# unsynchronized/gr-amps

Hardware: AMD Instinct MI355X
Metric: AMPS RECC Manchester symbols demodulated+decoded per second (real-time channels = value/0.02); achieved HBM GB/s vs peak (higher is better)
Workload: dtype f32

## Files before the change

gr_amps_amd/csrc/recc_decode.hip.h:

```cpp
#pragma once
#include <hip/hip_runtime.h>
#include <stdint.h>
#include "amps_recc.h"
#include "amps_recc_numerics.h"
#include "recc_devmem.hip.h"
#include "recc_record_host.h"

namespace amps {

struct Gf64Tables {
    uint8_t exp[128];
    uint8_t log[64];
};
constexpr Gf64Tables make_gf64()
{
    Gf64Tables t{};
    unsigned v = 1;
    for (int i = 0; i < 63; i++) {
        t.exp[i] = (uint8_t)v;
        t.exp[i + 63] = (uint8_t)v;
        t.log[v] = (uint8_t)i;
        v <<= 1;
        if (v & 0x40) v ^= 0x43;
    }
    t.exp[126] = t.exp[0];
    t.exp[127] = t.exp[1];
    t.log[0] = 0;
    return t;
}
struct SynMasks { uint64_t m1[6], m3[6]; };
constexpr SynMasks make_syn_masks()
{
    SynMasks s{};
    const Gf64Tables t = make_gf64();
    for (int e = 0; e < 63; e++)
        for (int k = 0; k < 6; k++) {
            if ((t.exp[e] >> k) & 1) s.m1[k] |= 1ull << e;
            if ((t.exp[(3 * e) % 63] >> k) & 1) s.m3[k] |= 1ull << e;
        }
    return s;
}
static constexpr SynMasks k_syn = make_syn_masks();

__device__ __forceinline__ unsigned gf_xtime(unsigned a)
{
    a <<= 1;
    return a ^ ((a & 0x40u) ? 0x43u : 0u);
}
__device__ __forceinline__ unsigned gf_mul(unsigned a, unsigned b)
{
    unsigned r = 0;
#pragma unroll
    for (int i = 0; i < 6; i++) { r ^= ((b >> i) & 1u) ? a : 0u; a = gf_xtime(a); }
    return r;
}
__device__ __forceinline__ unsigned gf_inv(unsigned a)
{
    const unsigned a2 = gf_mul(a, a), a4 = gf_mul(a2, a2), a8 = gf_mul(a4, a4), a16 = gf_mul(a8, a8), a32 = gf_mul(a16, a16);
    return gf_mul(gf_mul(gf_mul(a2, a4), gf_mul(a8, a16)), a32);
}
__device__ __forceinline__ unsigned gf_div(unsigned a, unsigned b) { return gf_mul(a, gf_inv(b)); }

struct BchResult {
    int ok;
    int nflip;
    int e[3];
};

__device__ __forceinline__ BchResult bch63_decode_packed(uint64_t w)
{
    BchResult r;
    r.ok = 0; r.nflip = 0; r.e[0] = r.e[1] = r.e[2] = -1;
    unsigned S1 = 0, S3 = 0;
#pragma unroll
    for (int k = 0; k < 6; k++) {
        S1 |= (unsigned)(__popcll(w & k_syn.m1[k]) & 1) << k;
        S3 |= (unsigned)(__popcll(w & k_syn.m3[k]) & 1) << k;
    }
    if ((S1 | S3) == 0) { r.ok = 1; return r; }
    int found = 0, e0 = -1, e1 = -1, e2 = -1;
    auto take = [&](bool root, int j) {
        const int pos = (63 - j) % 63;
        e0 = (root && found == 0) ? pos : e0;
        e1 = (root && found == 1) ? pos : e1;
        e2 = (root && found == 2) ? pos : e2;
        found += (root && found < 3) ? 1 : 0;
    };
    if (S1 != 0) {
        const unsigned S1cube = gf_mul(gf_mul(S1, S1), S1);
        const unsigned delta = S3 ^ S1cube;
        if (delta == 0) {
            unsigned p = 1;
            int lg = 0;
#pragma unroll 1
            for (int j = 0; j < 63; j++) { if (p == S1) lg = j; p = gf_xtime(p); }
            r.ok = 1; r.nflip = 1; r.e[0] = lg;
            return r;
        }
        const unsigned c2 = gf_div(delta, S1);
        unsigned a = S1, b = c2;
#pragma unroll 1
        for (int j = 0; j < 63; j++) {
            take((1u ^ a ^ b) == 0, j);
            a = gf_xtime(a);
            b = gf_xtime(gf_xtime(b));
        }
        r.e[0] = e0; r.e[1] = e1; r.e[2] = e2;
        if (found == 2) { r.ok = 1; r.nflip = 2; }
        return r;
    }
    {
        unsigned c = S3;
#pragma unroll 1
        for (int j = 0; j < 63; j++) {
            take((1u ^ c) == 0, j);
            c = gf_xtime(gf_xtime(gf_xtime(c)));
        }
        r.e[0] = e0; r.e[1] = e1; r.e[2] = e2;
        if (found == 3) { r.ok = 1; r.nflip = 3; }
    }
    return r;
}

__device__ __forceinline__ BchResult bch_short_decode(const uint8_t *bits, int nbits)
{
    uint64_t w = 0;
    for (int i = 0; i < nbits; i++) w |= (uint64_t)(bits[i] & 1u) << (nbits - 1 - i);
    return bch63_decode_packed(w);
}

__device__ __forceinline__ BchResult bch4836_decode(const uint8_t *bits) { return bch_short_decode(bits, 48); }

__device__ __forceinline__ BchResult bch4836_decode_aligned(const uint8_t *bits)
{
    const uint64_t *p = (const uint64_t *)bits;
    uint64_t w = 0;
#pragma unroll
    for (int c = 0; c < 6; c++) w |= ((p[c] * 0x8040201008040201ull) >> 56) << (40 - 8 * c);
    return bch63_decode_packed(w);
}

__device__ __forceinline__ void bch_short_encode(const uint8_t *msg, int k, uint8_t *cw)
{
    unsigned rem = 0;
    for (int j = 0; j < k; j++) {
        unsigned fb = ((rem >> 11) & 1u) ^ (msg[j] & 1u);
        rem = (rem << 1) & 0xfffu;
        if (fb) rem ^= 0x539u;
        cw[j] = msg[j] & 1u;
    }
    for (int j = 0; j < 12; j++) cw[k + j] = (uint8_t)((rem >> (11 - j)) & 1u);
}

__device__ __forceinline__ unsigned getbits(const uint8_t *b, int n)
{
    unsigned v = 0;
    for (int i = 0; i < n; i++) v = (v << 1) | (b[i] & 1u);
    return v;
}

__device__ __forceinline__ void extract_min_3(unsigned val, char *out)
{
    unsigned m2 = val + 111;
    unsigned dig = m2 % 10;
    out[2] = (char)('0' + dig);
    if (dig == 0) m2 -= 10; else m2 -= dig;
    dig = (m2 % 100) / 10;
    out[1] = (char)('0' + dig);
    if (dig == 0) m2 -= 100; else m2 -= (m2 % 100);
    dig = m2 / 100;
    if (dig > 9) dig = 0;
    out[0] = (char)('0' + dig);
}

constexpr int BOFF = 1;
struct DecodeCore {
    alignas(8) uint8_t bits[1696];
    uint64_t packed[7];
    uint32_t bad[8];
    uint32_t nonbin;
    int8_t   ok[35];
    int8_t   flip[35][3];
    int8_t   rr[8];
    int8_t   dly[AMPS_TRACK_BLOCKS];
    amps_recc_burst_t rec;
};
struct DecodeScratch {
    DecodeCore k;
    uint8_t sym[AMPS_RECC_CAPTURE_SYMS + 2];
};

struct BlockSync { static __device__ __forceinline__ void sync() { __syncthreads(); } };
struct WaveSync {
    static __device__ __forceinline__ void sync()
    {
        __builtin_amdgcn_fence(__ATOMIC_RELEASE, "wavefront");
        __builtin_amdgcn_wave_barrier();
        __builtin_amdgcn_fence(__ATOMIC_ACQUIRE, "wavefront");
    }
};

__device__ __forceinline__ void decode_core_begin(DecodeCore &s, int lane)
{
    if (lane < 8) s.bad[lane] = 0;
    if (lane == 8) s.nonbin = 0;
    for (int i = lane; i < (int)(sizeof(amps_recc_burst_t) / 4); i += 64) ((uint32_t *)&s.rec)[i] = 0;
}

template <class Sync>
__device__ __forceinline__ void manchester_from_sym(DecodeCore &s, const uint8_t *sym, int lane)
{
    decode_core_begin(s, lane);
    Sync::sync();
    const uint16_t *s16 = (const uint16_t *)sym;
#pragma unroll 9
    for (int it = 0; it < 27; it++) {
        const int k = lane + 64 * it;
        if (k < 1687) {
            const unsigned pr = s16[k];
            const unsigned sa = pr & 0xffu, sb = pr >> 8;
            const bool nonbin = (sa | sb) > 1u;
            const bool same = sa == sb;
            const unsigned bit = nonbin ? 0u : (same ? (sa ^ 1u) : sb);
            s.bits[BOFF + k] = (uint8_t)bit;
            if (nonbin) atomicOr(&s.nonbin, 1u);
            if (nonbin || same) atomicAdd(&s.bad[k < 7 ? 0 : 1 + (k - 7) / 240], 1u);
        }
    }
    Sync::sync();
}

constexpr int TRACK_PRE_BITS = AMPS_RECC_TRIGGER_SYMS / 2;
__host__ __device__ constexpr uint32_t capture_lead(uint32_t sps) { return sps * (AMPS_RECC_TRIGGER_SYMS - 1) + AMPS_TRACK_BLOCKS; }
__device__ __forceinline__ uint64_t capture_first_word(uint64_t nc, uint32_t sps)
{
    const uint64_t lead = capture_lead(sps);
    return (nc > lead ? nc - lead : 0ull) >> 6;
}
__device__ __forceinline__ uint32_t wave_sum_u32(uint32_t v)
{
    v += (uint32_t)__builtin_amdgcn_update_dpp(0, (int)v, 0xB1, 0xf, 0xf, true);
    v += (uint32_t)__builtin_amdgcn_update_dpp(0, (int)v, 0x4E, 0xf, 0xf, true);
    v += (uint32_t)__builtin_amdgcn_update_dpp(0, (int)v, 0x124, 0xf, 0xf, true);
    v += (uint32_t)__builtin_amdgcn_update_dpp(0, (int)v, 0x128, 0xf, 0xf, true);
    v += (uint32_t)__builtin_amdgcn_update_dpp(0, (int)v, 0x142, 0xa, 0xf, false);
    v += (uint32_t)__builtin_amdgcn_update_dpp(0, (int)v, 0x143, 0xc, 0xf, false);
    return (uint32_t)__builtin_amdgcn_readlane((int)v, 63);
}
template <class Sync, bool TWO = false>
__device__ __forceinline__ void manchester_from_ring(DecodeCore &s, const uint64_t *ring, uint64_t nc, uint64_t w0, uint32_t sps, int lane, bool track,
                                                     bool keep_delays = true)
{
    constexpr int EARLY = TWO ? 2 : 1;
    decode_core_begin(s, lane);
    Sync::sync();
    const uint32_t *r32 = (const uint32_t *)ring;
    const int32_t base = (int32_t)(nc - (w0 << 6));
    const uint32_t midmask = (1u << (sps - 1)) - 1u;
    uint32_t f_lo = 0u, f_hi = 0u, f_sh = 0u;
    int dly = 0, dly_fetched = 0;
    uint32_t badacc = 0u;
    auto fetch = [&](int k, int d, bool on) {
        const uint32_t na = (uint32_t)(base + (int32_t)sps * (2 * k + 1) + d - EARLY);
        const uint32_t q = on ? na >> 5 : 0u;
        f_lo = r32[q]; f_hi = r32[q + 1]; f_sh = na & 31u;
    };
    auto measure = [&](uint32_t w, bool on) {
        const uint32_t sa = w & 1u, sb = (w >> sps) & 1u;
        const uint32_t mid = (w >> 1) & midmask;
        const uint32_t cnt = (uint32_t)__popc(sa ? mid : (~mid & midmask));
        const uint32_t contrib = (on && sa != sb) ? ((cnt | (1u << 10)) << (sa ? 0 : 16)) : 0u;
        const uint32_t tot = wave_sum_u32(contrib);
        const int sum1 = (int)(tot & 0x3ffu), n1 = (int)((tot >> 10) & 0x3fu), sum0 = (int)((tot >> 16) & 0x3ffu), n0 = (int)(tot >> 26);
        const int E1 = 2 * sum1 - (int)(sps - 1) * n1, E0 = 2 * sum0 - (int)(sps - 1) * n0;
        const int lhs = E1 * n0 + E0 * n1, rhs = 2 * n0 * n1;
        if (rhs > 0) dly += lhs > rhs ? 1 : lhs < -rhs ? -1 : 0;
    };
    auto choose2 = [&](uint32_t w, bool on) -> int {
        const uint32_t e = w ^ (w >> 2);
        const uint32_t contrib = on ? ((~e & 1u) | ((~e & 2u) << 7) | ((~e & 4u) << 14)) : 0u;
        const uint32_t tot = wave_sum_u32(contrib);
        const uint32_t vm = tot & 0xffu, v0 = (tot >> 8) & 0xffu, vp = tot >> 16;
        int mv = 0;
        uint32_t best = v0;
        if (vm < v0) { mv = -1; best = vm; }
        if (vp < v0 && vp < best) mv = 1;
        return mv;
    };
    {
        const int k = -TRACK_PRE_BITS + lane;
        const bool on = lane < TRACK_PRE_BITS;
        const int32_t nas = base + (int32_t)sps * (2 * k + 1) - 1;
        const uint32_t na = nas < 0 ? 0u : (uint32_t)nas, q = on ? na >> 5 : 0u;
        const int32_t sh = -nas - 1;
        const uint32_t w = nas >= 0 ? __builtin_amdgcn_alignbit(r32[q + 1], r32[q], na & 31u) >> 1
                                    : sh >= 32 ? ~0u : ((r32[0] << (uint32_t)sh) | ((1u << (uint32_t)sh) - 1u));
        fetch(lane, 0, lane < 7 + AMPS_RECC_WORD_BITS);
        if constexpr (TWO) {
            const uint32_t w2 = nas >= 0 ? __builtin_amdgcn_alignbit(r32[q + 1], r32[q], na & 31u)
                                         : sh + 1 >= 32 ? ~0u : ((r32[0] << (uint32_t)(sh + 1)) | ((1u << (uint32_t)(sh + 1)) - 1u));
            if (track) dly += choose2(w2, on);
            if (lane == 0 && keep_delays) s.dly[0] = (int8_t)dly;
        } else {
        if (lane == 0 && keep_delays) s.dly[0] = 0;
        if (track) measure(w, on);
        }
    }
    {
        const int k = lane;
        const bool on = lane < 7 + AMPS_RECC_WORD_BITS;
        uint32_t w = __builtin_amdgcn_alignbit(f_hi, f_lo, f_sh) >> (uint32_t)(dly + 1);
        const int d1 = dly;
        fetch(7 + AMPS_RECC_WORD_BITS + lane, d1, lane < AMPS_RECC_WORD_BITS);
        if constexpr (TWO) {
            const int mv = track ? choose2(w, on) : 0;
            dly += mv;
            w >>= (uint32_t)(mv + 1);
        }
        if (lane == 0 && keep_delays) s.dly[1] = (int8_t)dly;
        const uint32_t sa = w & 1u, sb = (w >> sps) & 1u;
        if (on) s.bits[BOFF + k] = (uint8_t)(sa == sb ? (sa ^ 1u) : sb);
        const uint64_t bad = __ballot(on && sa == sb);
        if (lane == 0) s.bad[0] = (uint32_t)__popcll(bad & 0x7full);
        badacc = (uint32_t)__popcll(bad >> 7);
        if constexpr (!TWO) { if (track) measure(w, on); }
        dly_fetched = d1;
    }
    const bool on48 = lane < AMPS_RECC_WORD_BITS;
    uint8_t *bitp = &s.bits[BOFF + 7 + AMPS_RECC_WORD_BITS + lane];
    int kn = 7 + 2 * AMPS_RECC_WORD_BITS + lane;
    int rep = 1, word = 0;
#pragma unroll 1
    for (int b = 2; b < AMPS_TRACK_BLOCKS; b++) {
        uint32_t w = __builtin_amdgcn_alignbit(f_hi, f_lo, f_sh) >> (uint32_t)(dly - dly_fetched + 1);
        dly_fetched = dly;
        fetch(kn, dly, on48 && b + 1 < AMPS_TRACK_BLOCKS);
        kn += AMPS_RECC_WORD_BITS;
        if constexpr (TWO) {
            const int mv = track ? choose2(w, on48) : 0;
            dly += mv;
            w >>= (uint32_t)(mv + 1);
        }
        if (lane == 0 && keep_delays) s.dly[b] = (int8_t)dly;
        const uint32_t sa = w & 1u, sb = (w >> sps) & 1u;
        if (on48) *bitp = (uint8_t)(sa == sb ? (sa ^ 1u) : sb);
        bitp += AMPS_RECC_WORD_BITS;
        badacc += (uint32_t)__popcll(__ballot(on48 && sa == sb));
        if (++rep == AMPS_RECC_REPEATS) {
            if (lane == 0) s.bad[1 + word] = badacc;
            badacc = 0u; rep = 0; word++;
        }
        if constexpr (!TWO) { if (track) measure(w, on48); }
    }
    Sync::sync();
}

__device__ __forceinline__ void decode_core_store(const DecodeCore &s, amps_recc_burst_t *__restrict__ out, int lane)
{
    for (int i = lane; i < (int)(sizeof(amps_recc_burst_t) / 4); i += 64) ((uint32_t *)out)[i] = ((const uint32_t *)&s.rec)[i];
}

__device__ __forceinline__ void decode_core_store_packed(const DecodeCore &s, uint32_t *__restrict__ out, int lane)
{
    const uint32_t *rec = (const uint32_t *)&s.rec;
    if (lane < PACKED_RECORD_BYTES / 4) {
        uint32_t v;
        if (lane < 13) v = rec[lane];
        else if (lane >= 32) v = rec[REC_TAIL_OFF / 4 + (lane - 32)];
        else {
            const uint32_t *src = rec + (lane < 24 ? REC_RAW_OFF / 4 + 8 * (lane - 13) : REC_DEC_OFF / 4 + 8 * (lane - 24));
            v = 0u;
#pragma unroll
            for (int j = 0; j < 8; j++) {
                v |= ((((src[j] & 0x01010101u) * 0x01020408u) >> 24) & 0xfu) << (4 * j);
            }
        }
        out[lane] = v;
    }
}

struct NoTl { __device__ __forceinline__ void mark(int) {} };
template <class Sync, class Tl = NoTl>
__device__ __forceinline__ void decode_core_wave(DecodeCore &s, uint32_t channel, uint64_t position,
                                                 amps_recc_burst_t *__restrict__ out, bool majority, int lane, Tl tl = Tl())
{
    amps_recc_burst_t &o = s.rec;
    if (!majority) {
        if (lane < 35) {
            const int w = lane / 5, r = lane % 5;
            BchResult br = bch4836_decode_aligned(&s.bits[BOFF + 7 + 240 * w + 48 * r]);
            s.ok[lane] = (int8_t)br.ok;
            s.flip[lane][0] = (int8_t)br.e[0];
            s.flip[lane][1] = (int8_t)br.e[1];
            s.flip[lane][2] = (int8_t)br.e[2];
        }
        Sync::sync();
        tl.mark(1);
        if (lane < 7) {
            const int w = lane;
            int r = 0, ok = 0;
            for (; r < 5; r++) if (s.ok[w * 5 + r]) { ok = 1; break; }
            o.valid[w] = (uint8_t)ok;
            o.first_valid_rep[w] = (uint8_t)r;
            o.manch_bad[w] = (uint16_t)s.bad[1 + w];
            s.rr[w] = (int8_t)(ok ? r : 4);
        }
        for (int i = lane; i < 7 * 48; i += 64) o.word_raw[i / 48][i % 48] = s.bits[BOFF + 7 + 240 * (i / 48) + (i % 48)];
        Sync::sync();
        tl.mark(2);
        for (int i = lane; i < 7 * 36; i += 64) {
            const int w = i / 36, b = i % 36;
            o.word_dec[w][b] = s.bits[BOFF + 7 + 240 * w + 48 * s.rr[w] + b];
        }
        Sync::sync();
        tl.mark(3);
        if (lane < 7 && o.valid[lane]) {
            const int w = lane;
            for (int f = 0; f < 3; f++) {
                int e = s.flip[w * 5 + s.rr[w]][f];
                if (e >= 12 && e <= 47) o.word_dec[w][47 - e] ^= 1u;
            }
        }
    } else {
        for (int i = lane; i < 7 * 48; i += 64) {
            const int w = i / 48, b = i % 48;
            int cnt = 0;
            for (int r = 0; r < 5; r++) cnt += s.bits[BOFF + 7 + 240 * w + 48 * r + b];
            o.word_raw[w][b] = (uint8_t)(cnt >= 3);
        }
        Sync::sync();
        if (lane < 7) {
            const int w = lane;
            BchResult br = bch4836_decode(o.word_raw[w]);
            int ok = br.ok;
            for (int f = 0; f < 3; f++) if (br.e[f] >= 48) ok = 0;
            o.valid[w] = (uint8_t)ok;
            int agree = 0;
            for (int r = 0; r < 5; r++) {
                unsigned diff = 0;
#pragma unroll 8
                for (int b = 0; b < 48; b++) diff |= (unsigned)(s.bits[BOFF + 7 + 240 * w + 48 * r + b] ^ o.word_raw[w][b]);
                agree += diff == 0;
            }
            o.first_valid_rep[w] = (uint8_t)agree;
            o.manch_bad[w] = (uint16_t)s.bad[1 + w];
            for (int i = 0; i < 36; i++) o.word_dec[w][i] = o.word_raw[w][i];
            if (ok) for (int f = 0; f < 3; f++) { int e = br.e[f]; if (e >= 12 && e <= 47) o.word_dec[w][47 - e] ^= 1u; }
        }
    }
    if (lane < 7) o.dcc[lane] = s.bits[BOFF + lane];
    Sync::sync();
    tl.mark(4);
    for (int w = 0; w < 7; w++) {
        const uint8_t *src = majority ? o.word_dec[w] : o.word_raw[w];
        const unsigned bit = lane < 36 ? (src[lane] & 1u) : 0u;
        const uint64_t m = __ballot(bit != 0);
        if (lane == 0) s.packed[w] = __brevll(m);
    }
    Sync::sync();
    tl.mark(5);

    if (lane == 0) {
        o.channel = channel;
        o.position = position;
        o.flags = s.nonbin ? AMPS_BURST_FLAG_NONBINARY : 0u;
        o.dcc_bad = (uint8_t)s.bad[0];
        bool used_ok = true;
        auto W = [&](int w) -> uint64_t { used_ok = used_ok && o.valid[w]; return s.packed[w]; };
        auto fld = [](uint64_t wp, int off, int n) -> unsigned { return (unsigned)((wp >> (64 - off - n)) & ((1ull << n) - 1ull)); };
        const uint64_t A = W(0), B = W(1);
        if (majority) {
            const unsigned d = getbits(o.dcc, 7);
            const bool good = __popc(d ^ 0x00u) <= 1 || __popc(d ^ 0x1fu) <= 1 || __popc(d ^ 0x63u) <= 1 || __popc(d ^ 0x7cu) <= 1;
            if (!good) o.flags |= AMPS_BURST_FLAG_DCC_INVALID;
        }
        o.a_F = (uint8_t)fld(A, 0, 1); o.a_NAWC = (uint8_t)fld(A, 1, 3);
        o.a_T = (uint8_t)fld(A, 4, 1); o.a_S = (uint8_t)fld(A, 5, 1); o.a_E = (uint8_t)fld(A, 6, 1); o.a_ER = (uint8_t)fld(A, 7, 1);
        o.a_SCM = (uint8_t)fld(A, 8, 4); o.a_MIN1 = fld(A, 12, 24);
        o.b_F = (uint8_t)fld(B, 0, 1); o.b_NAWC = (uint8_t)fld(B, 1, 3);
        o.b_MSG_TYPE = (uint8_t)fld(B, 4, 5); o.b_ORDQ = (uint8_t)fld(B, 9, 3);
        o.b_ORDER = (uint8_t)fld(B, 12, 5); o.b_LT = (uint8_t)fld(B, 17, 1); o.b_EP = (uint8_t)fld(B, 18, 1);
        o.b_SCM4 = (uint8_t)fld(B, 19, 1); o.b_MPCI = (uint8_t)fld(B, 20, 2); o.b_SDCC1 = (uint8_t)fld(B, 22, 2);
        o.b_SDCC2 = (uint8_t)fld(B, 24, 2); o.b_MIN2 = (uint16_t)fld(B, 26, 10);
        extract_min_3(o.b_MIN2, o.min);
        extract_min_3((o.a_MIN1 >> 14) & 0x3ff, o.min + 3);
        unsigned thous = (o.a_MIN1 >> 10) & 0xf;
        if (thous > 9) thous = 0;
        o.min[6] = (char)('0' + thous);
        extract_min_3(o.a_MIN1 & 0x3ff, o.min + 7);

        const bool zero_order = (o.b_ORDER == 0 && o.b_ORDQ == 0 && o.b_MSG_TYPE == 0);
        if (!o.valid[0]) o.msg_class = AMPS_MSG_INVALID_WORD_A;
        else if (!o.a_E) o.msg_class = AMPS_MSG_E_ZERO;
        else if (o.a_T == 0 && zero_order) o.msg_class = AMPS_MSG_PAGE_RESPONSE;
        else if (o.a_T == 1 && o.b_ORDER == 0xd) {
            o.msg_class = AMPS_MSG_REGISTRATION;
            o.has_esn = o.a_S;
            if (o.a_S && o.a_NAWC > 1) {
                const uint64_t Cw = W(2);
                o.esn = fld(Cw, 4, 32);
                uint8_t nawc = (uint8_t)(o.a_NAWC - 2);
                if ((uint8_t)fld(Cw, 1, 3) != nawc) o.flags |= AMPS_BURST_FLAG_WORDC_NAWC_MISMATCH;
            }
        } else if (o.a_T == 1 && (o.a_NAWC > 2 || zero_order)) {
            uint8_t nawc = o.a_NAWC;
            unsigned next = 2;
            o.has_esn = o.a_S;
            if (o.a_S) {
                const uint64_t Cw = W(next++);
                o.esn = fld(Cw, 4, 32);
                nawc = (uint8_t)(o.a_NAWC - 2);
                if ((uint8_t)fld(Cw, 1, 3) != nawc) o.flags |= AMPS_BURST_FLAG_WORDC_NAWC_MISMATCH;
            }
            if (nawc < 1 || nawc > 4) o.msg_class = AMPS_MSG_BAD_NAWC;
            else {
                o.msg_class = AMPS_MSG_ORIGINATION;
                int dl = 0;
                for (; nawc > 0; nawc--) {
                    unsigned digs = fld(W(next++), 4, 32);
                    for (int i = 0; i < 8; i++) {
                        unsigned v = (digs >> 28) & 0xf;
                        if (v == 0) break;
                        if (v >= 13) { o.flags |= AMPS_BURST_FLAG_BAD_DIGIT; break; }
                        o.dialed[dl++] = v <= 9 ? (char)('0' + v) : v == 10 ? '0' : v == 11 ? '*' : '#';
                        digs <<= 4;
                    }
                    o.n_called_words++;
                }
            }
        } else o.msg_class = AMPS_MSG_UNKNOWN;
        if (majority && !used_ok && o.msg_class >= AMPS_MSG_PAGE_RESPONSE) o.msg_class = AMPS_MSG_INVALID_WORD_A;
    }
    Sync::sync();
    tl.mark(6);
    if (out) decode_core_store(s, out, lane);
    tl.mark(7);
}

__device__ __forceinline__ void decode_burst_wave(DecodeScratch &s, uint32_t channel, uint64_t position,
                                                  amps_recc_burst_t *__restrict__ out, bool majority = false)
{
    const int lane = threadIdx.x & 63;
    manchester_from_sym<BlockSync>(s.k, s.sym, lane);
    decode_core_wave<BlockSync>(s.k, channel, position, out, majority, lane);
}

__global__ __launch_bounds__(256) void bch_encode_words_kernel(const uint8_t *msg, uint32_t n, int k, uint8_t *cw)
{
    for (uint32_t i = blockIdx.x * 256 + threadIdx.x; i < n; i += gridDim.x * 256) {
        unsigned rem = 0;
        for (int j = 0; j < k; j++) {
            const unsigned bit = msg[(uint64_t)i * k + j] & 1u;
            const unsigned fb = ((rem >> 11) & 1u) ^ bit;
            rem = (rem << 1) & 0xfffu;
            if (fb) rem ^= 0x539u;
            cw[(uint64_t)i * (k + 12) + j] = (uint8_t)bit;
        }
        for (int j = 0; j < 12; j++) cw[(uint64_t)i * (k + 12) + k + j] = (uint8_t)((rem >> (11 - j)) & 1u);
    }
}
__global__ __launch_bounds__(256) void bch_decode_words_kernel(const uint8_t *cw, uint32_t n, int k, uint8_t *msg, uint8_t *valid,
                                                               uint8_t *nerr)
{
    const int nb = k + 12;
    for (uint32_t i = blockIdx.x * 256 + threadIdx.x; i < n; i += gridDim.x * 256) {
        uint64_t w = 0;
        for (int j = 0; j < nb; j++) w |= (uint64_t)(cw[(uint64_t)i * nb + j] & 1u) << (nb - 1 - j);
        const uint64_t raw = w;
        BchResult r = bch63_decode_packed(w);
        int ok = r.ok;
#pragma unroll
        for (int f = 0; f < 3; f++) {
            const int e = r.e[f];
            if (e >= nb) ok = 0;
            else if (r.ok && e >= 0) w ^= 1ull << e;
        }
        const uint64_t out = ok ? w : raw;
        for (int j = 0; j < k; j++) msg[(uint64_t)i * k + j] = (uint8_t)((out >> (nb - 1 - j)) & 1ull);
        valid[i] = (uint8_t)ok;
        nerr[i] = (uint8_t)(ok ? r.nflip : 0xff);
    }
}

struct BchScratch { DevBuf<uint8_t> in, out, val, err; };
inline int bch_grow(DevBuf<uint8_t> &b, size_t need)
{
    if (need <= b.capacity()) return 0;
    return b.reserve(need < 4096 ? 4096 : need + need / 2);
}
inline int bch_stage_in(BchScratch &b, hipStream_t s, const uint8_t *in, size_t nin, int mem, const uint8_t **din)
{
    if (mem == AMPS_MEM_DEVICE) { *din = in; return 0; }
    if (int rc = bch_grow(b.in, nin)) return rc;
    if (hipMemcpyAsync(b.in.get(), in, nin, hipMemcpyHostToDevice, s) != hipSuccess) return -EIO;
    *din = b.in.get();
    return 0;
}

}
```

gr_amps_amd/csrc/recc_resolve.hip.h:

```cpp
#pragma once
#include "recc_decode.hip.h"
#include "recc_bits.hip.h"

namespace amps {

struct ResolveArgs {
    const uint64_t *det;
    const uint32_t *detcount;
    uint32_t max_chunks, det_cap;
    uint32_t tiles_per_channel, span;
    uint32_t sps;
    uint64_t n_proc;
    uint64_t *next_allowed;
    uint64_t *pending;
    uint32_t *status;
    const uint64_t *gring;
    uint32_t ring_mask, ring_words;
    uint32_t cap_words;
    amps_recc_burst_t *records;
    uint32_t *nrecords;
    uint32_t rec_cap;
    uint32_t majority;
    uint32_t track;
    uint8_t *burst_syms;
    unsigned long long *done_blocks;
    uint32_t *hdr_host;
    uint64_t *capq;
    uint32_t *capq_count;
    uint32_t capq_cap;
    uint32_t search_P;
    uint32_t search_tol;
    uint32_t *zero1, *zero2;
    unsigned long long *tl;
};
#ifdef RESOLVE_TIMELINE
#define RTL(k) do { if (a.tl && tid == 0) a.tl[(size_t)blockIdx.x * 24 + (k)] = __builtin_amdgcn_s_memtime(); } while (0)
#else
#define RTL(k) do { } while (0)
#endif

constexpr int CAP_WAVES = 4;
__host__ __device__ constexpr uint32_t resolve_cap_stride(uint32_t cap_words) { return (uint32_t)((sizeof(DecodeCore) + 7) / 8) + cap_words; }
inline uint32_t resolve_cap_words(uint32_t sps) { return (AMPS_RECC_CAPTURE_SYMS * sps + sps + capture_lead(sps) + AMPS_TRACK_BLOCKS) / 64 + 4; }
inline size_t resolve_dyn_lds(uint32_t sps) { return (size_t)CAP_WAVES * resolve_cap_stride(resolve_cap_words(sps)) * 8; }

#ifdef RESOLVE_TIMELINE
struct RtlStamps {
    unsigned long long *dst;
    __device__ __forceinline__ void mark(int k) { if (dst) dst[k] = __builtin_amdgcn_s_memtime(); }
};
#else
typedef NoTl RtlStamps;
#endif
__device__ __forceinline__ void capture_gather_wave(const ResolveArgs &a, uint32_t c, uint64_t nc, uint64_t *scratch, int lane, RtlStamps tl = RtlStamps())
{
    uint64_t *s_ring = scratch + (sizeof(DecodeCore) + 7) / 8;
    const uint64_t *ring = a.gring + (uint64_t)c * a.ring_words;
    const uint64_t w0 = capture_first_word(nc, a.sps);
    const int nw = (int)(((nc + (uint64_t)a.sps * (AMPS_RECC_CAPTURE_SYMS + 1) + AMPS_TRACK_BLOCKS + 32) >> 6) - w0) + 1;
    for (int i0 = 0; i0 < nw; i0 += 512) {
        uint64_t v[8];
#pragma unroll
        for (int u = 0; u < 8; u++) {
            const int i = i0 + 64 * u + lane;
            v[u] = i < nw ? ring[(w0 + (uint64_t)i) & a.ring_mask] : 0ull;
        }
#pragma unroll
        for (int u = 0; u < 8; u++) {
            const int i = i0 + 64 * u + lane;
            if (i < nw) s_ring[i] = v[u];
        }
    }
    WaveSync::sync();
    tl.mark(8);
}
template <bool TWO>
__device__ __forceinline__ void capture_decode_wave(const ResolveArgs &a, uint32_t c, uint64_t nc, uint64_t *scratch, int lane, RtlStamps tl = RtlStamps())
{
    DecodeCore &k = *(DecodeCore *)scratch;
    const uint64_t *s_ring = scratch + (sizeof(DecodeCore) + 7) / 8;
    const uint64_t w0 = capture_first_word(nc, a.sps);
    manchester_from_ring<WaveSync, TWO>(k, s_ring, nc, w0, a.sps, lane, a.track != 0, a.burst_syms != nullptr);
    tl.mark(0);
    decode_core_wave<WaveSync>(k, c, nc, nullptr, a.majority != 0, lane, tl);
}
__device__ __forceinline__ void capture_store_wave(const ResolveArgs &a, uint64_t nc, uint32_t slot, const uint64_t *scratch, int lane)
{
    const DecodeCore &k = *(const DecodeCore *)scratch;
    decode_core_store_packed(k, (uint32_t *)((uint8_t *)a.records + (size_t)slot * PACKED_RECORD_BYTES), lane);
    if (a.burst_syms) {
        const uint64_t *s_ring = scratch + (sizeof(DecodeCore) + 7) / 8;
        const uint64_t w0 = capture_first_word(nc, a.sps);
        uint32_t *dst = (uint32_t *)(a.burst_syms + (uint64_t)slot * PACKED_BURST_BYTES);
        for (int dw = lane; dw < PACKED_BURST_BYTES / 4; dw += 64) {
            uint32_t word = 0u;
            for (int j = 0; j < 32; j++) {
                const int i = 32 * dw + j;
                if (i < AMPS_RECC_CAPTURE_SYMS) {
                    const int kb = i >> 1, blk = kb < 7 + AMPS_RECC_WORD_BITS ? 1 : 2 + (kb - 7 - AMPS_RECC_WORD_BITS) / AMPS_RECC_WORD_BITS;
                    const uint64_t n = (uint64_t)((int64_t)nc + (int64_t)a.sps * (i + 1) + k.dly[blk]);
                    word |= (uint32_t)((s_ring[(n >> 6) - w0] >> (n & 63)) & 1ull) << j;
                }
            }
            dst[dw] = word;
        }
    }
}

constexpr uint32_t DONE_GROUPS = 32;
__device__ __forceinline__ unsigned long long count_done(unsigned long long *p, uint32_t done, unsigned long long reserved)
{
    return __hip_atomic_fetch_add(p, (reserved << 32) | done, __ATOMIC_RELAXED, __HIP_MEMORY_SCOPE_AGENT);
}
__device__ __forceinline__ void publish_header(uint32_t *nrecords , uint32_t *status,
                                               volatile uint32_t *hdr_host, unsigned long long launch_total)
{
    const uint32_t total = nrecords[2] + (uint32_t)launch_total;
    nrecords[2] = total;
    hdr_host[0] = total;
    hdr_host[1] = __hip_atomic_load(status, __ATOMIC_RELAXED, __HIP_MEMORY_SCOPE_AGENT);
}

constexpr int RESOLVE_THREADS = 256;
constexpr int RESOLVE_THREADS_WIDE = 1024;
constexpr int RESOLVE_LDS_HITS = 512;
constexpr int RESOLVE_LDS_HITS_WIDE = 2048;

constexpr int RESOLVE_SEARCH_CAP = 320;
template <int THREADS, int HITS, bool TWO = false, int SEARCH = 0, bool STOL = false>
__global__ __launch_bounds__(THREADS, 4) void recc_resolve_kernel(ResolveArgs a)
{
    static_assert(SEARCH == 0 || (THREADS == 256 && (SEARCH == 2 || SEARCH == 3)), "the search stage runs in the narrow kernel, at the wideband seam's rates");
    __shared__ __attribute__((aligned(16))) uint32_t s_sw[SEARCH ? 4 : 1][SEARCH ? 8 + 64 * 4 : 1];
    __shared__ uint64_t s_sdet[SEARCH ? 4 : 1][SEARCH ? RESOLVE_SEARCH_CAP : 1];
    __shared__ uint32_t s_scnt[4];
    __shared__ uint64_t s_hits[HITS];
    __shared__ uint32_t s_scan[THREADS / 64];
    __shared__ uint64_t s_acc[HITS + 1];
    __shared__ uint8_t  s_head[HITS], s_accf[HITS];
    __shared__ uint64_t s_na_out, s_pend;
    __shared__ uint32_t s_total, s_nacc, s_base;
    extern __shared__ uint64_t s_cap[];
    const int c = blockIdx.x, tid = threadIdx.x;
    const int wv = __builtin_amdgcn_readfirstlane(tid >> 6), lane = tid & 63;
    RTL(0);
    const uint64_t span_hold = (uint64_t)a.sps * (AMPS_RECC_CAPTURE_SYMS + AMPS_RECC_TRIGGER_SYMS);
    const uint64_t span_done = (uint64_t)a.sps * (AMPS_RECC_CAPTURE_SYMS + 1) + (a.track ? AMPS_TRACK_BLOCKS : 0);
    uint64_t next_allowed = a.next_allowed[c];
    uint64_t pend = a.pending[c];
    if constexpr (SEARCH != 0) {
        if (blockIdx.x == 0 && tid == 0) {
            if (a.zero1) *a.zero1 = 0u;
            if (a.zero2) { a.zero2[0] = 0u; a.zero2[1] = 0u; a.zero2[2] = 0u; }
        }
        const uint32_t Tc = (a.search_P + TILE - 1) / TILE;
        const uint32_t t_lo = (uint32_t)((uint64_t)Tc * (uint32_t)wv / 4u), t_hi = (uint32_t)((uint64_t)Tc * ((uint32_t)wv + 1u) / 4u);
        uint32_t nd = 0;
        if (t_hi > t_lo)
            nd = bits_search_segment<SEARCH, STOL>(a.gring + (uint64_t)c * a.ring_words, a.ring_words, a.n_proc - a.search_P, a.search_P, a.search_tol, a.status,
                                                   t_lo, t_hi, s_sw[wv], s_sdet[wv], (uint32_t)RESOLVE_SEARCH_CAP, lane);
        if (lane == 0) s_scnt[wv] = nd < (uint32_t)RESOLVE_SEARCH_CAP ? nd : (uint32_t)RESOLVE_SEARCH_CAP;
        __syncthreads();
    }
    const uint32_t n_first = [&]() -> uint32_t {
        if constexpr (SEARCH != 0) return (uint32_t)tid < 4u ? s_scnt[tid] : 0u;
        const uint64_t gs0 = (uint64_t)c * a.tiles_per_channel;
        const uint32_t nch = (uint32_t)((gs0 + a.tiles_per_channel - 1) / a.span - gs0 / a.span) + 1;
        return (uint32_t)tid < nch ? a.detcount[(uint64_t)c * a.max_chunks + (uint32_t)tid] : 0u;
    }();
    auto centre = [](uint64_t ei) -> uint64_t { return (ei >> 8) + (uint32_t)(ei & 0xff) / 2; };

    uint32_t reserved = 0;
    auto flush = [&]() {
        __syncthreads();
        const uint32_t m = s_nacc;
        if (!a.capq) reserved += m;
        if (m && a.capq) {
            if (tid == 0) s_base = atomicAdd(a.capq_count, m);
            __syncthreads();
            const uint32_t base = s_base;
            for (uint32_t i = tid; i < m; i += THREADS) {
                if (base + i < a.capq_cap) a.capq[base + i] = ((uint64_t)c << CAPQ_POS_BITS) | (s_acc[i] & ((1ull << CAPQ_POS_BITS) - 1));
                else atomicOr(a.status, 2u);
            }
            __syncthreads();
        } else if (m) {
            for (uint32_t i0 = 0; i0 < m; i0 += CAP_WAVES) {
                const uint32_t i = i0 + (uint32_t)wv;
                const bool mine = wv < CAP_WAVES && i < m;
                uint64_t *scr = s_cap + (size_t)wv * resolve_cap_stride(a.cap_words);
#ifdef RESOLVE_TIMELINE
                RtlStamps st{ (a.tl && tid == 0) ? a.tl + (size_t)blockIdx.x * 24 + 8 : nullptr };
#else
                RtlStamps st;
#endif
                if (mine) capture_gather_wave(a, (uint32_t)c, s_acc[i], scr, lane, st);
                if (i0 == 0) {
                    __syncthreads();
                    if (tid == THREADS - 1) s_base = atomicAdd(a.nrecords, m);
                }
                if (mine) capture_decode_wave<TWO>(a, (uint32_t)c, s_acc[i], scr, lane, st);
                RTL(3);
                __syncthreads();
                RTL(4);
                if (mine) {
                    const uint32_t slot = s_base + i;
                    if (slot < a.rec_cap) capture_store_wave(a, s_acc[i], slot, scr, lane);
                    else if (lane == 0) { atomicOr(a.status, 4u); __threadfence(); }
                }
                __syncthreads();
            }
        }
    };
    if (tid == 0) s_nacc = 0;
    if (pend != ~0ull && pend + span_done < a.n_proc) {
        if (tid == 0) { s_acc[0] = pend; s_nacc = 1; }
        pend = ~0ull;
    }

    const uint64_t gs = (uint64_t)c * a.tiles_per_channel;
    const uint32_t nchunks = SEARCH != 0 ? 4u : (uint32_t)((gs + a.tiles_per_channel - 1) / a.span - gs / a.span) + 1;
    const uint32_t *cnt = SEARCH != 0 ? s_scnt : a.detcount + (uint64_t)c * a.max_chunks;
    const uint64_t *det = SEARCH != 0 ? &s_sdet[0][0] : a.det + (uint64_t)c * a.max_chunks * a.det_cap;
    const uint32_t det_cap = SEARCH != 0 ? (uint32_t)RESOLVE_SEARCH_CAP : a.det_cap;

    for (uint32_t cb = 0; cb < nchunks; cb += THREADS) {
        const uint32_t ch = cb + tid;
        const uint32_t n = cb == 0 ? n_first : (ch < nchunks ? cnt[ch] : 0u);
        uint32_t incl = n;
#pragma unroll
        for (int off = 1; off < 64; off <<= 1) {
            const uint32_t y = (uint32_t)__shfl_up((int)incl, off);
            if (lane >= off) incl += y;
        }
        if (lane == 63) s_scan[wv] = incl;
        __syncthreads();
        for (int w = 0; w < wv; w++) incl += s_scan[w];
        const uint32_t excl = incl - n;
        if (tid == THREADS - 1) s_total = incl;
        __syncthreads();
        const uint32_t batch_total = s_total;
        RTL(1);
        const uint64_t *d = det + (uint64_t)ch * det_cap;
        for (uint32_t win = 0; win == 0 || win < batch_total; win += HITS) {
            if (tid == 0) { s_pend = ~0ull; s_na_out = next_allowed; }
            for (uint32_t i = 0; i < n; i++) {
                const uint32_t g = excl + i;
                if (g >= win && g < win + HITS) s_hits[g - win] = d[i];
            }
            __syncthreads();
            const uint32_t total = batch_total - win < (uint32_t)HITS ? batch_total - win : (uint32_t)HITS;
            for (uint32_t j = tid; j < total; j += THREADS)
                s_head[j] = (j == 0) || ((s_hits[j] >> 8) >= (s_hits[j - 1] >> 8) + 128 + span_hold && (s_hits[j] >> 8) >= next_allowed);
            __syncthreads();
            for (uint32_t j = tid; j < total; j += THREADS) {
                if (!s_head[j]) continue;
                uint64_t na = j == 0 ? next_allowed : 0ull;
                uint32_t k = j;
                do {
                    const uint64_t ei = s_hits[k];
                    const bool acc = (ei >> 8) >= na;
                    if (acc) na = centre(ei) + span_hold;
                    s_accf[k] = (uint8_t)acc;
                    k++;
                } while (k < total && !s_head[k]);
                if (k == total) s_na_out = na;
            }
            __syncthreads();
            for (uint32_t j = tid; j < total; j += THREADS) {
                if (!s_accf[j]) continue;
                const uint64_t nc = centre(s_hits[j]);
                if (nc + span_done < a.n_proc) s_acc[atomicAdd(&s_nacc, 1u)] = nc;
                else s_pend = nc;
            }
            __syncthreads();
            next_allowed = s_na_out;
            if (s_pend != ~0ull) pend = s_pend;
            RTL(2);
            flush();
            RTL(5);
            if (tid == 0) s_nacc = 0;
            __syncthreads();
        }
    }
    if (tid == 0) { a.next_allowed[c] = next_allowed; a.pending[c] = pend; }
    if (tid == 0 && !a.capq) {
        RTL(6);
        const uint32_t ng = gridDim.x < DONE_GROUPS ? gridDim.x : DONE_GROUPS;
        const uint32_t g = blockIdx.x % DONE_GROUPS;
        const uint32_t gsize = (gridDim.x - g + DONE_GROUPS - 1) / DONE_GROUPS;
        const unsigned long long gv = count_done(a.done_blocks + 1 + g, 1u, reserved);
        if ((uint32_t)gv == gsize - 1) {
            const unsigned long long gtot = (gv >> 32) + reserved;
            atomicExch(a.done_blocks + 1 + g, 0ull);
            const unsigned long long tv = count_done(a.done_blocks, 1u, gtot);
            if ((uint32_t)tv == ng - 1) {
                publish_header(a.nrecords, a.status, a.hdr_host, (tv >> 32) + gtot);
                atomicExch(a.done_blocks, 0ull);
            }
        }
        RTL(7);
    }
}

inline bool resolve_uses_queue(uint32_t n_channels) { return n_channels < 64; }
template <bool TWO = false>
__global__ __launch_bounds__(64) void recc_capture_kernel(ResolveArgs a)
{
    extern __shared__ uint64_t s_cap[];
    const int lane = threadIdx.x;
    uint32_t ncap = *a.capq_count;
    if (ncap > a.capq_cap) ncap = a.capq_cap;
    uint32_t reserved = 0;
    for (uint32_t q = blockIdx.x; q < ncap; q += gridDim.x) {
        reserved++;
        const uint64_t e = a.capq[q];
        const uint32_t c = (uint32_t)(e >> CAPQ_POS_BITS);
        const uint64_t nc = e & ((1ull << CAPQ_POS_BITS) - 1);
        capture_gather_wave(a, c, nc, s_cap, lane);
        uint32_t slot = 0;
        if (lane == 0) slot = atomicAdd(a.nrecords, 1u);
        capture_decode_wave<TWO>(a, c, nc, s_cap, lane);
        slot = (uint32_t)__builtin_amdgcn_readfirstlane((int)slot);
        if (slot < a.rec_cap) capture_store_wave(a, nc, slot, s_cap, lane);
        else if (lane == 0) { atomicOr(a.status, 4u); __threadfence(); }
        WaveSync::sync();
    }
    const uint32_t nb = ncap < gridDim.x ? (ncap ? ncap : 1u) : gridDim.x;
    if (lane == 0 && blockIdx.x < nb) {
        const unsigned long long t = count_done(a.done_blocks, 1u, reserved);
        if ((uint32_t)t == nb - 1) {
            publish_header(a.nrecords, a.status, a.hdr_host, (t >> 32) + reserved);
            atomicExch(a.done_blocks, 0ull);
        }
    }
}

__global__ __launch_bounds__(64) void recc_decode_bursts_kernel(const uint8_t *bursts, const uint32_t *chan,
                                                                uint32_t nbursts, amps_recc_burst_t *out, uint32_t majority)
{
    __shared__ DecodeScratch s;
    const int lane = threadIdx.x;
    for (uint32_t q = blockIdx.x; q < nbursts; q += gridDim.x) {
        const uint8_t *b = bursts + (uint64_t)q * AMPS_RECC_CAPTURE_SYMS;
        for (int i = lane; i < AMPS_RECC_CAPTURE_SYMS; i += 64) s.sym[i] = b[i];
        __syncthreads();
        decode_burst_wave(s, chan ? chan[q] : 0u, 0ull, out + q, majority != 0);
        __syncthreads();
    }
}

}
```

Baseline: 228,500.

## Parallelize burst field decoding across wave lanes and drop shared scratch syncs

Replaces shared-memory staging of BCH results (ok/flip/rr/packed) with wave ballots and readlane broadcasts. This removes several wave barriers. The serial lane-0 field extraction, MIN digit conversion and dialed-digit decoding are spread across lanes, with each lane writing one record byte from constexpr shift and mask tables. It also adds timeline probe macros that only compile under RESOLVE_TIMELINE. The aim is to cut the single-lane serial tail of the decode, in exchange for more complex lane-indexed logic that must match the old semantics exactly, including digit-stop behaviour and the ESN and NAWC handling.

After: 229,200, median of 5. Within noise of the previous version (+0.3%).

```diff
diff --git a/gr_amps_amd/csrc/recc_decode.hip.h b/gr_amps_amd/csrc/recc_decode.hip.h
--- a/gr_amps_amd/csrc/recc_decode.hip.h
+++ b/gr_amps_amd/csrc/recc_decode.hip.h
@@ -176,12 +176,8 @@
 constexpr int BOFF = 1;
 struct DecodeCore {
     alignas(8) uint8_t bits[1696];
-    uint64_t packed[7];
     uint32_t bad[8];
     uint32_t nonbin;
-    int8_t   ok[35];
-    int8_t   flip[35][3];
-    int8_t   rr[8];
     int8_t   dly[AMPS_TRACK_BLOCKS];
     amps_recc_burst_t rec;
 };
@@ -379,48 +375,67 @@
     }
 }
 
+constexpr int FIELD_BYTES_A = 12, FIELD_BYTES = 26;
+struct FieldTables { uint64_t sh[4], mask[4]; };
+constexpr FieldTables make_field_tables()
+{
+    struct Fd { int off, n, byte; };
+    constexpr Fd f[FIELD_BYTES] = {
+        { 0, 1, 0 }, { 1, 3, 0 }, { 4, 1, 0 }, { 5, 1, 0 }, { 6, 1, 0 }, { 7, 1, 0 }, { 8, 4, 0 }, { 0, 0, 0 },
+        { 12, 24, 0 }, { 12, 24, 1 }, { 12, 24, 2 }, { 12, 24, 3 },
+        { 0, 1, 0 }, { 1, 3, 0 }, { 4, 5, 0 }, { 9, 3, 0 }, { 12, 5, 0 }, { 17, 1, 0 }, { 18, 1, 0 }, { 19, 1, 0 },
+        { 20, 2, 0 }, { 22, 2, 0 }, { 24, 2, 0 }, { 0, 0, 0 }, { 26, 10, 0 }, { 26, 10, 1 } };
+    FieldTables t{};
+    for (int i = 0; i < FIELD_BYTES; i++) {
+        const int left = f[i].n - 8 * f[i].byte;
+        if (left <= 0) continue;
+        t.sh[i / 8] |= (uint64_t)(64 - f[i].off - f[i].n + 8 * f[i].byte) << (8 * (i % 8));
+        t.mask[i / 8] |= (uint64_t)((1u << (left < 8 ? left : 8)) - 1u) << (8 * (i % 8));
+    }
+    return t;
+}
+static constexpr FieldTables k_fields = make_field_tables();
+static_assert(offsetof(amps_recc_burst_t, a_MIN1) == REC_TAIL_OFF + 8 && offsetof(amps_recc_burst_t, b_F) == REC_TAIL_OFF + FIELD_BYTES_A &&
+              offsetof(amps_recc_burst_t, b_MIN2) == REC_TAIL_OFF + 24 && offsetof(amps_recc_burst_t, b_MIN2) + 2 == REC_TAIL_OFF + FIELD_BYTES, "field bytes");
+
 struct NoTl { __device__ __forceinline__ void mark(int) {} };
 template <class Sync, class Tl = NoTl>
 __device__ __forceinline__ void decode_core_wave(DecodeCore &s, uint32_t channel, uint64_t position,
                                                  amps_recc_burst_t *__restrict__ out, bool majority, int lane, Tl tl = Tl())
 {
     amps_recc_burst_t &o = s.rec;
+    uint32_t vmask;
     if (!majority) {
-        if (lane < 35) {
-            const int w = lane / 5, r = lane % 5;
-            BchResult br = bch4836_decode_aligned(&s.bits[BOFF + 7 + 240 * w + 48 * r]);
-            s.ok[lane] = (int8_t)br.ok;
-            s.flip[lane][0] = (int8_t)br.e[0];
-            s.flip[lane][1] = (int8_t)br.e[1];
-            s.flip[lane][2] = (int8_t)br.e[2];
-        }
-        Sync::sync();
+        BchResult br;
+        br.ok = 0; br.nflip = 0; br.e[0] = br.e[1] = br.e[2] = -1;
+        if (lane < 35) br = bch4836_decode_aligned(&s.bits[BOFF + 7 + 240 * (lane / 5) + 48 * (lane % 5)]);
+        const uint64_t okm = __ballot(lane < 35 && br.ok != 0);
         tl.mark(1);
+        auto first_rep = [&](int w) -> int { const uint32_t m = (uint32_t)(okm >> (5 * w)) & 31u; return m ? __builtin_ctz(m) : 5; };
         if (lane < 7) {
-            const int w = lane;
-            int r = 0, ok = 0;
-            for (; r < 5; r++) if (s.ok[w * 5 + r]) { ok = 1; break; }
-            o.valid[w] = (uint8_t)ok;
-            o.first_valid_rep[w] = (uint8_t)r;
-            o.manch_bad[w] = (uint16_t)s.bad[1 + w];
-            s.rr[w] = (int8_t)(ok ? r : 4);
+            const int r = first_rep(lane);
+            o.valid[lane] = (uint8_t)(r < 5);
+            o.first_valid_rep[lane] = (uint8_t)r;
+            o.manch_bad[lane] = (uint16_t)s.bad[1 + lane];
+            o.dcc[lane] = s.bits[BOFF + lane];
         }
         for (int i = lane; i < 7 * 48; i += 64) o.word_raw[i / 48][i % 48] = s.bits[BOFF + 7 + 240 * (i / 48) + (i % 48)];
-        Sync::sync();
-        tl.mark(2);
         for (int i = lane; i < 7 * 36; i += 64) {
-            const int w = i / 36, b = i % 36;
-            o.word_dec[w][b] = s.bits[BOFF + 7 + 240 * w + 48 * s.rr[w] + b];
+            const int w = i / 36, b = i % 36, r = first_rep(w);
+            o.word_dec[w][b] = s.bits[BOFF + 7 + 240 * w + 48 * (r < 5 ? r : 4) + b];
         }
         Sync::sync();
         tl.mark(3);
-        if (lane < 7 && o.valid[lane]) {
-            const int w = lane;
+        if (lane < 35 && br.ok && lane % 5 == first_rep(lane / 5)) {
+#pragma unroll
             for (int f = 0; f < 3; f++) {
-                int e = s.flip[w * 5 + s.rr[w]][f];
-                if (e >= 12 && e <= 47) o.word_dec[w][47 - e] ^= 1u;
+                const int e = br.e[f];
+                if (e >= 12 && e <= 47) o.word_dec[lane / 5][47 - e] ^= 1u;
             }
         }
+        vmask = 0u;
+#pragma unroll
+        for (int w = 0; w < 7; w++) vmask |= (first_rep(w) < 5 ? 1u : 0u) << w;
     } else {
         for (int i = lane; i < 7 * 48; i += 64) {
             const int w = i / 48, b = i % 48;
@@ -429,10 +444,11 @@
             o.word_raw[w][b] = (uint8_t)(cnt >= 3);
         }
         Sync::sync();
+        int ok = 0;
         if (lane < 7) {
             const int w = lane;
             BchResult br = bch4836_decode(o.word_raw[w]);
-            int ok = br.ok;
+            ok = br.ok;
             for (int f = 0; f < 3; f++) if (br.e[f] >= 48) ok = 0;
             o.valid[w] = (uint8_t)ok;
             int agree = 0;
@@ -446,90 +462,115 @@
             o.manch_bad[w] = (uint16_t)s.bad[1 + w];
             for (int i = 0; i < 36; i++) o.word_dec[w][i] = o.word_raw[w][i];
             if (ok) for (int f = 0; f < 3; f++) { int e = br.e[f]; if (e >= 12 && e <= 47) o.word_dec[w][47 - e] ^= 1u; }
-        }
-    }
-    if (lane < 7) o.dcc[lane] = s.bits[BOFF + lane];
-    Sync::sync();
-    tl.mark(4);
-    for (int w = 0; w < 7; w++) {
-        const uint8_t *src = majority ? o.word_dec[w] : o.word_raw[w];
-        const unsigned bit = lane < 36 ? (src[lane] & 1u) : 0u;
-        const uint64_t m = __ballot(bit != 0);
-        if (lane == 0) s.packed[w] = __brevll(m);
-    }
-    Sync::sync();
+            o.dcc[w] = s.bits[BOFF + w];
+        }
+        vmask = (uint32_t)__ballot(lane < 7 && ok != 0);
+        Sync::sync();
+        tl.mark(4);
+    }
+    const int pw = lane < 7 ? lane : 6;
+    uint64_t pk = 0;
+    {
+        const uint32_t *src = (const uint32_t *)(majority ? o.word_dec[pw] : o.word_raw[pw]);
+#pragma unroll
+        for (int j = 0; j < 9; j++) pk |= (uint64_t)((((src[j] & 0x01010101u) * 0x08040201u) >> 24) & 0xfu) << (60 - 4 * j);
+    }
+    const uint32_t dccm = (uint32_t)__ballot(lane < 7 && (s.bits[BOFF + pw] & 1u));
+    uint64_t P[7];
+#pragma unroll
+    for (int w = 0; w < 7; w++)
+        P[w] = ((uint64_t)(uint32_t)__builtin_amdgcn_readlane((int)(uint32_t)(pk >> 32), w) << 32) | (uint32_t)__builtin_amdgcn_readlane((int)(uint32_t)pk, w);
     tl.mark(5);
 
+    auto fld = [](uint64_t wp, int off, int n) -> unsigned { return (unsigned)((wp >> (64 - off - n)) & ((1ull << n) - 1ull)); };
+    const uint64_t A = P[0], B = P[1];
+    if (lane < FIELD_BYTES) {
+        const int g = lane >> 3, q = 8 * (lane & 7);
+        const uint64_t tsh = g == 0 ? k_fields.sh[0] : g == 1 ? k_fields.sh[1] : g == 2 ? k_fields.sh[2] : k_fields.sh[3];
+        const uint64_t tmk = g == 0 ? k_fields.mask[0] : g == 1 ? k_fields.mask[1] : g == 2 ? k_fields.mask[2] : k_fields.mask[3];
+        const uint64_t wp = lane < FIELD_BYTES_A ? A : B;
+        ((uint8_t *)&o)[REC_TAIL_OFF + lane] = (uint8_t)((unsigned)(wp >> ((unsigned)(tsh >> q) & 0xffu)) & (unsigned)(tmk >> q) & 0xffu);
+    }
+    const unsigned MIN1 = fld(A, 12, 24), MIN2 = fld(B, 26, 10);
+    if (lane < 3) extract_min_3(lane == 0 ? MIN2 : lane == 1 ? (MIN1 >> 14) & 0x3ffu : MIN1 & 0x3ffu, o.min + (lane == 0 ? 0 : lane == 1 ? 3 : 7));
+    if (lane == 3) {
+        unsigned thous = (MIN1 >> 10) & 0xfu;
+        if (thous > 9) thous = 0;
+        o.min[6] = (char)('0' + thous);
+    }
+
+    unsigned flags = s.nonbin ? AMPS_BURST_FLAG_NONBINARY : 0u;
+    if (majority) {
+        const unsigned d = __brev(dccm) >> 25;
+        const bool good = __popc(d ^ 0x00u) <= 1 || __popc(d ^ 0x1fu) <= 1 || __popc(d ^ 0x63u) <= 1 || __popc(d ^ 0x7cu) <= 1;
+        if (!good) flags |= AMPS_BURST_FLAG_DCC_INVALID;
+    }
+    const unsigned a_NAWC = fld(A, 1, 3), a_T = fld(A, 4, 1), a_S = fld(A, 5, 1), a_E = fld(A, 6, 1);
+    const unsigned b_MSG_TYPE = fld(B, 4, 5), b_ORDQ = fld(B, 9, 3), b_ORDER = fld(B, 12, 5);
+    const bool zero_order = (b_ORDER == 0 && b_ORDQ == 0 && b_MSG_TYPE == 0);
+    unsigned used = 3u, msg_class, has_esn = 0u;
+    bool read_c = false;
+    int first_called = 0, n_called = 0;
+    if (!(vmask & 1u)) msg_class = AMPS_MSG_INVALID_WORD_A;
+    else if (!a_E) msg_class = AMPS_MSG_E_ZERO;
+    else if (a_T == 0 && zero_order) msg_class = AMPS_MSG_PAGE_RESPONSE;
+    else if (a_T == 1 && b_ORDER == 0xd) {
+        msg_class = AMPS_MSG_REGISTRATION;
+        has_esn = a_S;
+        read_c = a_S && a_NAWC > 1;
+    } else if (a_T == 1 && (a_NAWC > 2 || zero_order)) {
+        unsigned nawc = a_NAWC;
+        has_esn = a_S;
+        read_c = a_S != 0;
+        if (a_S) nawc = (a_NAWC - 2u) & 0xffu;
+        if (nawc < 1 || nawc > 4) msg_class = AMPS_MSG_BAD_NAWC;
+        else {
+            msg_class = AMPS_MSG_ORIGINATION;
+            first_called = a_S ? 3 : 2;
+            n_called = (int)nawc;
+        }
+    } else msg_class = AMPS_MSG_UNKNOWN;
+    unsigned esn = 0u;
+    if (read_c) {
+        used |= 4u;
+        esn = fld(P[2], 4, 32);
+        if (fld(P[2], 1, 3) != ((a_NAWC - 2u) & 0xffu)) flags |= AMPS_BURST_FLAG_WORDC_NAWC_MISMATCH;
+    }
+    if (n_called) {
+        used |= ((1u << n_called) - 1u) << first_called;
+        const bool mine = lane >= first_called && lane < first_called + n_called;
+        const uint32_t digs = (uint32_t)(pk >> 28);
+        int n = 8;
+        bool bad = false;
+#pragma unroll
+        for (int i = 7; i >= 0; i--) {
+            const unsigned v = (digs >> (28 - 4 * i)) & 0xfu;
+            if (v == 0 || v >= 13) { n = i; bad = v >= 13; }
+        }
+        n = mine ? n : 0;
+        int at = 0;
+#pragma unroll
+        for (int w = 2; w < 6; w++) {
+            const int nw = __builtin_amdgcn_readlane(n, w);
+            at += lane > w ? nw : 0;
+        }
+        if (__ballot(mine && bad)) flags |= AMPS_BURST_FLAG_BAD_DIGIT;
+#pragma unroll
+        for (int i = 0; i < 8; i++) {
+            const unsigned v = (digs >> (28 - 4 * i)) & 0xfu;
+            if (i < n) o.dialed[at + i] = v <= 9 ? (char)('0' + v) : v == 10 ? '0' : v == 11 ? '*' : '#';
+        }
+    }
+    if (majority && (vmask & used) != used && msg_class >= AMPS_MSG_PAGE_RESPONSE) msg_class = AMPS_MSG_INVALID_WORD_A;
     if (lane == 0) {
         o.channel = channel;
         o.position = position;
-        o.flags = s.nonbin ? AMPS_BURST_FLAG_NONBINARY : 0u;
+        o.flags = flags;
         o.dcc_bad = (uint8_t)s.bad[0];
-        bool used_ok = true;
-        auto W = [&](int w) -> uint64_t { used_ok = used_ok && o.valid[w]; return s.packed[w]; };
-        auto fld = [](uint64_t wp, int off, int n) -> unsigned { return (unsigned)((wp >> (64 - off - n)) & ((1ull << n) - 1ull)); };
-        const uint64_t A = W(0), B = W(1);
-        if (majority) {
-            const unsigned d = getbits(o.dcc, 7);
-            const bool good = __popc(d ^ 0x00u) <= 1 || __popc(d ^ 0x1fu) <= 1 || __popc(d ^ 0x63u) <= 1 || __popc(d ^ 0x7cu) <= 1;
-            if (!good) o.flags |= AMPS_BURST_FLAG_DCC_INVALID;
-        }
-        o.a_F = (uint8_t)fld(A, 0, 1); o.a_NAWC = (uint8_t)fld(A, 1, 3);
-        o.a_T = (uint8_t)fld(A, 4, 1); o.a_S = (uint8_t)fld(A, 5, 1); o.a_E = (uint8_t)fld(A, 6, 1); o.a_ER = (uint8_t)fld(A, 7, 1);
-        o.a_SCM = (uint8_t)fld(A, 8, 4); o.a_MIN1 = fld(A, 12, 24);
-        o.b_F = (uint8_t)fld(B, 0, 1); o.b_NAWC = (uint8_t)fld(B, 1, 3);
-        o.b_MSG_TYPE = (uint8_t)fld(B, 4, 5); o.b_ORDQ = (uint8_t)fld(B, 9, 3);
-        o.b_ORDER = (uint8_t)fld(B, 12, 5); o.b_LT = (uint8_t)fld(B, 17, 1); o.b_EP = (uint8_t)fld(B, 18, 1);
-        o.b_SCM4 = (uint8_t)fld(B, 19, 1); o.b_MPCI = (uint8_t)fld(B, 20, 2); o.b_SDCC1 = (uint8_t)fld(B, 22, 2);
-        o.b_SDCC2 = (uint8_t)fld(B, 24, 2); o.b_MIN2 = (uint16_t)fld(B, 26, 10);
-        extract_min_3(o.b_MIN2, o.min);
-        extract_min_3((o.a_MIN1 >> 14) & 0x3ff, o.min + 3);
-        unsigned thous = (o.a_MIN1 >> 10) & 0xf;
-        if (thous > 9) thous = 0;
-        o.min[6] = (char)('0' + thous);
-        extract_min_3(o.a_MIN1 & 0x3ff, o.min + 7);
-
-        const bool zero_order = (o.b_ORDER == 0 && o.b_ORDQ == 0 && o.b_MSG_TYPE == 0);
-        if (!o.valid[0]) o.msg_class = AMPS_MSG_INVALID_WORD_A;
-        else if (!o.a_E) o.msg_class = AMPS_MSG_E_ZERO;
-        else if (o.a_T == 0 && zero_order) o.msg_class = AMPS_MSG_PAGE_RESPONSE;
-        else if (o.a_T == 1 && o.b_ORDER == 0xd) {
-            o.msg_class = AMPS_MSG_REGISTRATION;
-            o.has_esn = o.a_S;
-            if (o.a_S && o.a_NAWC > 1) {
-                const uint64_t Cw = W(2);
-                o.esn = fld(Cw, 4, 32);
-                uint8_t nawc = (uint8_t)(o.a_NAWC - 2);
-                if ((uint8_t)fld(Cw, 1, 3) != nawc) o.flags |= AMPS_BURST_FLAG_WORDC_NAWC_MISMATCH;
-            }
-        } else if (o.a_T == 1 && (o.a_NAWC > 2 || zero_order)) {
-            uint8_t nawc = o.a_NAWC;
-            unsigned next = 2;
-            o.has_esn = o.a_S;
-            if (o.a_S) {
-                const uint64_t Cw = W(next++);
-                o.esn = fld(Cw, 4, 32);
-                nawc = (uint8_t)(o.a_NAWC - 2);
-                if ((uint8_t)fld(Cw, 1, 3) != nawc) o.flags |= AMPS_BURST_FLAG_WORDC_NAWC_MISMATCH;
-            }
-            if (nawc < 1 || nawc > 4) o.msg_class = AMPS_MSG_BAD_NAWC;
-            else {
-                o.msg_class = AMPS_MSG_ORIGINATION;
-                int dl = 0;
-                for (; nawc > 0; nawc--) {
-                    unsigned digs = fld(W(next++), 4, 32);
-                    for (int i = 0; i < 8; i++) {
-                        unsigned v = (digs >> 28) & 0xf;
-                        if (v == 0) break;
-                        if (v >= 13) { o.flags |= AMPS_BURST_FLAG_BAD_DIGIT; break; }
-                        o.dialed[dl++] = v <= 9 ? (char)('0' + v) : v == 10 ? '0' : v == 11 ? '*' : '#';
-                        digs <<= 4;
-                    }
-                    o.n_called_words++;
-                }
-            }
-        } else o.msg_class = AMPS_MSG_UNKNOWN;
-        if (majority && !used_ok && o.msg_class >= AMPS_MSG_PAGE_RESPONSE) o.msg_class = AMPS_MSG_INVALID_WORD_A;
+        o.esn = esn;
+        o.has_esn = (uint8_t)has_esn;
+        o.msg_class = (uint8_t)msg_class;
+        o.n_called_words = (uint8_t)n_called;
     }
     Sync::sync();
     tl.mark(6);
diff --git a/gr_amps_amd/csrc/recc_resolve.hip.h b/gr_amps_amd/csrc/recc_resolve.hip.h
--- a/gr_amps_amd/csrc/recc_resolve.hip.h
+++ b/gr_amps_amd/csrc/recc_resolve.hip.h
@@ -35,8 +35,15 @@
 };
 #ifdef RESOLVE_TIMELINE
 #define RTL(k) do { if (a.tl && tid == 0) a.tl[(size_t)blockIdx.x * 24 + (k)] = __builtin_amdgcn_s_memtime(); } while (0)
+#define RTL_WHERE() do { if (a.tl && tid == 0) { unsigned long long *tl_ = a.tl + (size_t)blockIdx.x * 24; \
+        tl_[17] = __builtin_amdgcn_s_getreg((20 << 0) | (0 << 6) | (3 << 11)) & 0xf; \
+        tl_[18] = __builtin_amdgcn_s_getreg((4 << 0) | (0 << 6) | (15 << 11)) & 0xffff; \
+        tl_[19] = __builtin_amdgcn_s_memrealtime(); } } while (0)
+#define RTL_REAL(k) do { if (a.tl && tid == 0) a.tl[(size_t)blockIdx.x * 24 + (k)] = __builtin_amdgcn_s_memrealtime(); } while (0)
 #else
 #define RTL(k) do { } while (0)
+#define RTL_WHERE() do { } while (0)
+#define RTL_REAL(k) do { } while (0)
 #endif
 
 constexpr int CAP_WAVES = 4;
@@ -144,6 +151,7 @@
     const int c = blockIdx.x, tid = threadIdx.x;
     const int wv = __builtin_amdgcn_readfirstlane(tid >> 6), lane = tid & 63;
     RTL(0);
+    RTL_WHERE();
     const uint64_t span_hold = (uint64_t)a.sps * (AMPS_RECC_CAPTURE_SYMS + AMPS_RECC_TRIGGER_SYMS);
     const uint64_t span_done = (uint64_t)a.sps * (AMPS_RECC_CAPTURE_SYMS + 1) + (a.track ? AMPS_TRACK_BLOCKS : 0);
     uint64_t next_allowed = a.next_allowed[c];
@@ -300,6 +308,7 @@
             }
         }
         RTL(7);
+        RTL_REAL(20);
     }
 }
 
```
